# fransiskusbudi/multimodal_segmentation_project

Hardware: AMD Instinct MI355X
Metric: 3D volumes/sec (96^3, 4-class) fwd+bwd per node (higher is better)
Workload: dtype bf16; 1 GPU; UNet3D(1->4, features 16/32/64/128) 96^3 patch, per-GPU batch 2, fwd + Dice/CE loss + bwd + AdamW + metrics, dropout 0.0; global_batch=2, parallelism=dp1, hipgraph=False

## Files before the change

multimodal_segmentation_project_amd/csrc/common.h:

```cpp
#pragma once
#include <hip/hip_runtime.h>
#include <stdint.h>

typedef __bf16 bf16;
typedef __attribute__((ext_vector_type(8))) __bf16 bf16x8;
typedef __attribute__((ext_vector_type(4))) __bf16 bf16x4;
typedef __attribute__((ext_vector_type(4))) float f32x4;
typedef __attribute__((ext_vector_type(16))) float f32x16;

enum { MI3D_F32 = 0, MI3D_BF16 = 1 };

void mi3d_set_error(const char* fmt, ...);
#define MI3D_CHECK_ARG(cond, ...)                 \
    do {                                          \
        if (!(cond)) {                            \
            mi3d_set_error(__VA_ARGS__);          \
            return -1;                            \
        }                                         \
    } while (0)
#define MI3D_HIP(call)                                                                   \
    do {                                                                                 \
        hipError_t e_ = (call);                                                          \
        if (e_ != hipSuccess) {                                                          \
            mi3d_set_error("%s failed: %s (%s:%d)", #call, hipGetErrorString(e_), __FILE__, __LINE__); \
            return (int)e_;                                                              \
        }                                                                                \
    } while (0)
#define MI3D_LAUNCH_CHECK() MI3D_HIP(hipGetLastError())
#define MI3D_TRY(expr)          \
    do {                        \
        int rc_ = (expr);       \
        if (rc_ != 0) return rc_; \
    } while (0)

#define MI3D_ROUTE_LIST(X)                                                                                          \
    X(no_planar, 0)                                     \
    X(no_persist, 0)                                \
    X(no_head_loss, 0)                      \
    X(no_pool_fuse, 0)                                           \
    X(no_small_bn, 0)       \
    X(no_defer_tail, 0)                                     \
    X(no_upbwd_carry, 0)      \
    X(no_fused_bwd, 0)         \
    X(no_fused_bwd_p, 0)                                          \
    X(no_fused_bwd_big, 0)                                              \
    X(no_fused_upbwd, 0)                   \
    X(conv8, 1)                                  \
    X(no_pool_splitk, 0)     \
    X(no_pool_pair, 0)       \
    X(wide_bn, 3)            \
    X(splitk_ticket, 1)
struct Mi3dRoutes {
#define MI3D_ROUTE_FIELD(name, dflt) int name = dflt;
    MI3D_ROUTE_LIST(MI3D_ROUTE_FIELD)
#undef MI3D_ROUTE_FIELD
};
const Mi3dRoutes& mi3d_routes();

#ifdef __HIPCC__
#define MI3D_HD __host__ __device__
// ... 89 lines not shown
```

multimodal_segmentation_project_amd/csrc/conv3_mfma.hip:

```cpp
#include <stdlib.h>

#include <type_traits>

#include <hip/hip_ext.h>

#include "mfma_tile.h"
#include "ops.h"
#include "slab_sum.h"

namespace {

constexpr int BLK = 256;

MI3D_HD constexpr int ktap(int mode, int s, int h) {
    if (mode == 0) return 2 * s + h;
    if (s < 12) {
        int dz = s / 4, k = s % 4;
        return k < 3 ? dz * 9 + k * 3 + h : dz * 9 + h * 3 + 2;
    }
    if (s == 12) return h * 9 + 8;
    return h == 0 ? 26 : 27;
}

__global__ void pack_mfma_kernel(const float* __restrict__ w, int Cin, int Cout, bf16* __restrict__ wf, bf16* __restrict__ wd,
                                 int mode_f, int mode_d) {
    int64_t n = (int64_t)Cin * Cout * 28;
    for (int64_t i = (int64_t)blockIdx.x * blockDim.x + threadIdx.x; i < 2 * n; i += (int64_t)gridDim.x * blockDim.x) {
        bool dg = i >= n;
        int64_t k = dg ? i - n : i;
        int j = k & 7; int lane = (k >> 3) & 63; int64_t r = k >> 9;
        int nob = (dg ? Cin : Cout) / 16;
// ... 547 lines not shown
            }
            __syncthreads();
            bn_row_write<COB, 8, false>(red, tk_rows, bid_.x, CoutTotal, cobBase * 16);
            return;
        }
    }
    float s1[COB][4], s2[COB][4];
#pragma unroll
    for (int c = 0; c < COB; c++)
#pragma unroll
        for (int j = 0; j < 4; j++) s1[c][j] = s2[c][j] = 0.f;
#pragma unroll
    for (int r = 0; r < MBW; r++)
        conv_epilogue<T, COB, STATS, true>(acc[r], bias, y, ycs, relu, n, z0 + zs, y0, x0, hb * MBW + r, vn, g, D, H, W, cobBase, s1, s2);
    if constexpr (STATS) bn_rows_reduce<COB, 8, false>(s1, s2, red, wave, vn, g, part, bid_.x, CoutTotal, cobBase * 16);
}

template <int COB, int NCH, bool STATS, bool EXT_LDS = false>
__device__ __forceinline__ void conv3_mfma_persist_body(Bid bid_, const bf16* __restrict__ x, int xcs,
                                                        const bf16* __restrict__ wp, const float* __restrict__ bias,
                                                        bf16* __restrict__ y, int ycs, int D, int H, int W,
                                                        int tilesZ, int tilesY, int tilesX, int ntiles,
                                                        float* __restrict__ part, Halves xh, Halves yh, char* ext_lds = nullptr,
                                                        int relu = 0) {
    using T = FullTile;
    using L = LdsP<COB, NCH>;
    constexpr int TZ = T::TZ, TY = T::TY, TX = T::TX, IY = T::IY, IX = T::IX, MB = T::MB;
    static_assert(T::BX == 16 && T::IXP == IX && MB == 8, "a lane's voxel is x position vn of M-block row r; rows are not padded");
    constexpr int NVOX = T::NVOX, NIT = T::pieces(BLK);
    constexpr int CoutTotal = COB * 16;
    constexpr int NWF = NCH * 14 * COB;
    bf16* xs; bf16* wl;
    float (*red)[COB][16][2];
    if constexpr (EXT_LDS) {
        xs = reinterpret_cast<bf16*>(ext_lds + L::xs);
        wl = reinterpret_cast<bf16*>(ext_lds + L::wl);
        red = reinterpret_cast<float (*)[COB][16][2]>(ext_lds + L::red);
    } else {
        __shared__ __attribute__((aligned(16))) bf16 xs_s[(L::wl - L::xs) / 2];
        __shared__ __attribute__((aligned(16))) bf16 wl_s[(L::red - L::wl) / 2];
        __shared__ float red_s[4][COB][16][2];
        static_assert(sizeof(xs_s) + sizeof(wl_s) + sizeof(red_s) == L::bytes, "the three arrays are the layout");
        xs = xs_s; wl = wl_s; red = red_s;
    }
    int lane = threadIdx.x & 63, wave = threadIdx.x >> 6;
    int vn = lane & 15, g = lane >> 4;
    int laneOff = ((vn * 16 + (g & 1) * 8) * 2) + wave * (IY * IX * 32);
// ... 10 lines not shown
    bool lastValid = threadIdx.x + (NIT - 1) * BLK < NVOX * 2;
    unsigned pk[(NIT + 1) / 2];
#pragma unroll
    for (int i = 0; i < (NIT + 1) / 2; i++) pk[i] = 0;
#pragma unroll
    for (int it = 0; it < NIT; it++) {
        int vox = (threadIdx.x + it * BLK) >> 1;
        int ix = vox % IX, t = vox / IX, iy = t % IY, iz = t / IY;
        if (iz > 7) iz = 7;
        pk[it >> 1] |= (unsigned)(ix | (iy << 5) | (iz << 9)) << ((it & 1) * 16);
    }
    float bv[COB][4];
#pragma unroll
    for (int c = 0; c < COB; c++)
#pragma unroll
        for (int j = 0; j < 4; j++) bv[c][j] = bias ? bias[c * 16 + g * 4 + j] : 0.f;
    float s1[COB][4], s2[COB][4];
#pragma unroll
    for (int c = 0; c < COB; c++)
#pragma unroll
        for (int j = 0; j < 4; j++) s1[c][j] = s2[c][j] = 0.f;

    bf16x8 sv[NIT];
    auto tile_origin = [&](int tile, int& n, int& z0, int& y0, int& x0) {
        int tz_ = tile % tilesZ; tile /= tilesZ;
        int ty_ = tile % tilesY; tile /= tilesY;
        int tx_ = tile % tilesX; n = tile / tilesX;
        z0 = tz_ * TZ; y0 = ty_ * TY; x0 = tx_ * TX;
    };
    auto load_pieces = [&](int tile, int chunk) {
        int n, z0, y0, x0;
        tile_origin(tile, n, z0, y0, x0);
        int64_t base = ((((int64_t)n * D + (z0 - 1)) * H + (y0 - 1)) * W + (x0 - 1)) * xcs + chunk * 16 +
                       (chunk >= xh.split ? xh.delta : 0);
        const bf16* xb = x + base;
        bool interior = z0 >= 1 && z0 + TZ + 1 <= D && y0 >= 1 && y0 + TY + 1 <= H && x0 >= 1 && x0 + TX + 1 <= W;
        if (interior) {
#pragma unroll
            for (int it = 0; it < NIT; it++) {
                if (it < NIT - 1 || lastValid) sv[it] = *reinterpret_cast<const bf16x8*>(xb + rel[it]);
            }
        } else {
#pragma unroll
            for (int it = 0; it < NIT; it++) {
                unsigned c = pk[it >> 1] >> ((it & 1) * 16);
                unsigned gz = (unsigned)(z0 - 1) + ((c >> 9) & 7u), gy = (unsigned)(y0 - 1) + ((c >> 5) & 15u),
                         gx = (unsigned)(x0 - 1) + (c & 31u);
                bool inb = (it < NIT - 1 || lastValid) && gz < (unsigned)D && gy < (unsigned)H && gx < (unsigned)W;
                sv[it] = bf16x8{0, 0, 0, 0, 0, 0, 0, 0};
                if (inb) sv[it] = *reinterpret_cast<const bf16x8*>(xb + rel[it]);
            }
        }
    };

    int tile = xcd_contig(bid_.x, bid_.gx);
    if (tile < ntiles) load_pieces(tile, 0);
    for (int i = threadIdx.x; i < NWF * 64; i += BLK)
        *reinterpret_cast<bf16x8*>(wl + i * 8) = *reinterpret_cast<const bf16x8*>(wp + (int64_t)i * 8);
    for (; tile < ntiles; tile += bid_.gx) {
        f32x4 acc[MB][COB];
#pragma unroll
        for (int r = 0; r < MB; r++)
#pragma unroll
            for (int c = 0; c < COB; c++) acc[r][c] = f32x4{0.f, 0.f, 0.f, 0.f};
#pragma unroll
        for (int ch = 0; ch < NCH; ch++) {
            __syncthreads();
#pragma unroll
            for (int it = 0; it < NIT; it++) {
                int idx = threadIdx.x + it * BLK;
                if (it < NIT - 1 || idx < NVOX * 2) *reinterpret_cast<bf16x8*>(xs + idx * 8) = sv[it];
            }
            __syncthreads();
            if (ch + 1 < NCH) load_pieces(tile, ch + 1);
            else if (tile + bid_.gx < ntiles) load_pieces(tile + bid_.gx, 0);
            auto W_ = [&](int s, int c) -> bf16x8 {
                return *reinterpret_cast<const bf16x8*>(wl + ((ch * 14 + s) * COB + c) * 512 + lane * 8);
            };
            const int hx = (g >> 1) * 32;
            const int hy = (g >> 1) * (IX * 32) + 64;
            const int hz = (g >> 1) * (IY * IX * 32) + (2 * IX + 2) * 32;
            bf16x8 F[10], G[8];
#pragma unroll
            for (int row = 0; row < 10; row++) F[row] = *reinterpret_cast<const bf16x8*>(xsb + laneOff + hx + row * (IX * 32));
#pragma unroll
            for (int dz = 0; dz < 3; dz++) {
#pragma unroll
                for (int r = 0; r < 8; r++)
                    G[r] = *reinterpret_cast<const bf16x8*>(xsb + laneOff + hy + (dz * IY + r) * (IX * 32));
#pragma unroll
                for (int dy = 0; dy < 3; dy++) {
                    bf16x8 wc_[COB];
#pragma unroll
                    for (int c = 0; c < COB; c++) wc_[c] = W_(dz * 4 + dy, c);
#pragma unroll
                    for (int r = 0; r < 8; r++)
#pragma unroll
                        for (int c = 0; c < COB; c++) acc[r][c] = mfma16(wc_[c], F[r + dy], acc[r][c]);
// ... 15 lines not shown
#pragma unroll
                        for (int c = 0; c < COB; c++) acc[r][c] = mfma16(wc_[c], G[r], acc[r][c]);
                }
            }
#pragma unroll
            for (int r = 0; r < 8; r++)
                G[r] = *reinterpret_cast<const bf16x8*>(xsb + laneOff + (2 * IY * IX + 2 * IX + 2) * 32 + r * (IX * 32));
            {
                bf16x8 wc_[COB];
#pragma unroll
                for (int c = 0; c < COB; c++) wc_[c] = W_(12, c);
#pragma unroll
                for (int r = 0; r < 8; r++)
#pragma unroll
                    for (int c = 0; c < COB; c++) acc[r][c] = mfma16(wc_[c], F[r], acc[r][c]);
#pragma unroll
                for (int c = 0; c < COB; c++) wc_[c] = W_(13, c);
#pragma unroll
                for (int r = 0; r < 8; r++)
#pragma unroll
                    for (int c = 0; c < COB; c++) acc[r][c] = mfma16(wc_[c], G[r], acc[r][c]);
            }
        }
        int n, z0, y0, x0;
        tile_origin(tile, n, z0, y0, x0);
        int gz = z0 + wave, gx = x0 + vn;
        bf16* yrow = y + ((((int64_t)n * D + gz) * H + y0) * W + gx) * ycs + g * 4;
        bool okzx = gz < D && gx < W;
        if (relu & 2) {
            bf16* ywide = y + ((((int64_t)n * D + gz) * H + y0 + (g & 1)) * W + gx) * ycs + (g >> 1) * 8;
#pragma unroll
            for (int r = 0; r < MB; r += 2) {
                const bool okw = okzx && (y0 + r + (g & 1)) < H;
#pragma unroll
                for (int c = 0; c < COB; c++) {
                    bf16x4 oa, ob;
#pragma unroll
                    for (int j = 0; j < 4; j++) {
                        float va = acc[r][c][j] + bv[c][j], vb = acc[r + 1][c][j] + bv[c][j];
                        if (relu & 1) { va = fmaxf(va, 0.f); vb = fmaxf(vb, 0.f); }
                        oa[j] = (bf16)va; ob[j] = (bf16)vb;
                        if (STATS) {
                            float qa = (okzx && (y0 + r) < H) ? (float)oa[j] : 0.f, qb = (okzx && (y0 + r + 1) < H) ? (float)ob[j] : 0.f;
                            s1[c][j] += qa; s2[c][j] = fmaf(qa, qa, s2[c][j]);
                            s1[c][j] += qb; s2[c][j] = fmaf(qb, qb, s2[c][j]);
                        }
                    }
                    u32x4 w = swap_halves16(oa, ob);
                    if (okw) *reinterpret_cast<u32x4*>(ywide + (int64_t)r * W * ycs + c * 16 + (c >= yh.split ? yh.delta : 0)) = w;
                }
            }
            continue;
        }
#pragma unroll
        for (int r = 0; r < MB; r++) {
            bool ok = okzx && (y0 + r) < H;
#pragma unroll
            for (int c = 0; c < COB; c++) {
                bf16x4 o = round4_masked<STATS>(acc[r][c], bv[c], relu, ok, s1[c], s2[c]);
                if (ok) *reinterpret_cast<bf16x4*>(yrow + (int64_t)r * W * ycs + c * 16 + (c >= yh.split ? yh.delta : 0)) = o;
            }
        }
    }
    if constexpr (STATS) bn_rows_reduce<COB, 4, true>(s1, s2, red, wave, vn, g, part, bid_.x, CoutTotal, 0);
}

template <int COB, int NCH, bool STATS>
__global__ __launch_bounds__(BLK, 2) void conv3_mfma_persist_kernel(const bf16* __restrict__ x, int xcs,
                                                                    const bf16* __restrict__ wp, const float* __restrict__ bias,
                                                                    bf16* __restrict__ y, int ycs, int D, int H, int W,
                                                                    int tilesZ, int tilesY, int tilesX, int ntiles,
                                                                    float* __restrict__ part, Halves xh, Halves yh, int relu) {
    conv3_mfma_persist_body<COB, NCH, STATS>(real_bid(), x, xcs, wp, bias, y, ycs, D, H, W, tilesZ, tilesY, tilesX, ntiles, part, xh, yh,
                                             nullptr, relu);
}

inline int device_cus() {
    static const int n = [] {
        int dev = 0, v = 0;
        if (hipGetDevice(&dev) != hipSuccess || hipDeviceGetAttribute(&v, hipDeviceAttributeMultiprocessorCount, dev) != hipSuccess || v < 8)
            v = 256;
        (void)hipGetLastError();
        return v;
    }();
    return n;
}
struct TimeHook { hipEvent_t e0 = nullptr, e1 = nullptr; int kind = -1, cin = 0, cout = 0; bool armed = false, fired = false; };
static thread_local TimeHook g_hook;
inline bool time_hook_take(int kind, int cin, int cout, hipEvent_t& e0, hipEvent_t& e1) {
    if (kind < 0 || !g_hook.armed || g_hook.kind != kind || g_hook.cin != cin || g_hook.cout != cout) return false;
    e0 = g_hook.e0; e1 = g_hook.e1;
    g_hook.armed = false; g_hook.fired = true;
    return true;
}
template <auto Kernel, typename... Args>
int launch_hooked(dim3 grid, dim3 block, size_t lds, hipStream_t s, int kind, int cin, int cout, Args... args) {
    if (lds) MI3D_SET_MAX_LDS_ONCE(Kernel, lds);
    hipEvent_t e0 = nullptr, e1 = nullptr;
    if (time_hook_take(kind, cin, cout, e0, e1)) hipExtLaunchKernelGGL(Kernel, grid, block, lds, s, e0, e1, 0, args...);
    else Kernel<<<grid, block, lds, s>>>(args...);
    MI3D_LAUNCH_CHECK();
    return 0;
}

inline bool persist_ok(int Cin, int Cout, Geo g) {
    int64_t nt = (int64_t)g.N * cdiv(g.D, 4) * cdiv(g.H, 8) * cdiv(g.W, 16);
    if (Cin == 16 && Cout == 32 && nt < 1024) return false;
    return g.W >= 32 && g.H >= 16 && ((Cin == 16 && Cout == 16) || (Cin == 32 && Cout == 16) || (Cin == 16 && Cout == 32)) &&
           !mi3d_routes().no_persist;
}
inline int persist_grid(int Cin, int Cout, Geo g) {
    int64_t nt = (int64_t)g.N * cdiv(g.D, 4) * cdiv(g.H, 8) * cdiv(g.W, 16);
    int want = 2 * device_cus();
    return (int)(nt < want ? nt : want);
}

__device__ __forceinline__ void splitk_finish_body(int blk, int nblk, const float* __restrict__ part, int ksplit, int64_t M, int C,
                                                   const float* __restrict__ bias, bf16* __restrict__ y, int ycs, int relu = 0) {
    int G8 = C / 8;
    int64_t total = M * G8;
    for (int64_t idx = (int64_t)blk * BLK + threadIdx.x; idx < total; idx += (int64_t)nblk * BLK) {
        int64_t v = idx / G8;
        int c0 = (int)(idx - v * G8) * 8;
        float a[8];
#pragma unroll
        for (int j = 0; j < 8; j++) a[j] = bias ? bias[c0 + j] : 0.f;
        for (int k = 0; k < ksplit; k++) {
            const float* p = part + ((int64_t)k * M + v) * C + c0;
            f32x4 u = *reinterpret_cast<const f32x4*>(p), w = *reinterpret_cast<const f32x4*>(p + 4);
            a[0] += u[0]; a[1] += u[1]; a[2] += u[2]; a[3] += u[3]; a[4] += w[0]; a[5] += w[1]; a[6] += w[2]; a[7] += w[3];
        }
        if (relu) {
// ... 118 lines not shown
bool conv3_mfma_fuses_stats(int Cin, int Cout, Geo g) { return pick_ksplit(Cin, Cout, g) == 1; }

bool conv3_mfma_halves_ok(int Cin, int Cout, Geo g) { return persist_ok(Cin, Cout, g); }

bool conv3_mfma_ticket_ok(int Cin, int Cout, Geo g) {
    if (!mi3d_routes().splitk_ticket || mi3d_routes().conv8 == 0 || big_geo(g) || persist_ok(Cin, Cout, g)) return false;
    if (pick_ksplit(Cin, Cout, g) <= 1) return false;
    const int64_t wgs = (int64_t)g.N * cdiv(g.D, 4) * cdiv(g.H, 8) * cdiv(g.W, 8) * (Cout / (Cout % 32 == 0 ? 32 : 16));
    return wgs <= CONV3_TK_COUNTERS;
}

int conv3_mfma_fwd(const void* x, int xcs, int Cin, const void* wp, const float* bias, void* y, int ycs, int Cout, Geo g,
                   float* part, float* skws, hipStream_t s, Halves xh, Halves yh, int* ks_deferred, int relu, int split_target,
                   float* tk_rows, int* tk_count) {
    if (ks_deferred) *ks_deferred = 0;
    MI3D_CHECK_ARG(!tk_rows || (conv3_mfma_ticket_ok(Cin, Cout, g) && skws && split_target == 0), "conv3_mfma_fwd: no split-K ticket for %d->%d here", Cin, Cout);
    MI3D_CHECK_ARG((!xh.on() && !yh.on()) || persist_ok(Cin, Cout, g), "conv3_mfma_fwd: planar halves need the persistent kernel");
    MI3D_CHECK_ARG(conv3_mfma_supported(Cin, Cout, xcs, ycs), "conv3_mfma_fwd: unsupported channels %d->%d", Cin, Cout);
    MI3D_CHECK_ARG(((uintptr_t)x % 16) == 0 && ((uintptr_t)y % 8) == 0, "conv3_mfma_fwd: misaligned tensors");
    const bf16* xp = (const bf16*)x; const bf16* w = (const bf16*)wp; bf16* yp = (bf16*)y;
    bool two = Cout % 32 == 0;
    if (persist_ok(Cin, Cout, g)) {
        int tz = cdiv(g.D, 4), ty = cdiv(g.H, 8), tx = cdiv(g.W, 16), nt = g.N * tz * ty * tx, grid = persist_grid(Cin, Cout, g);
        if (ycs % 8 == 0 && ((uintptr_t)y % 16) == 0 && yh.delta % 8 == 0) relu |= 2;
        auto launch = [&](auto cob, auto nch) -> int {
            constexpr int COB = decltype(cob)::value, NCH = decltype(nch)::value;
            if (part)
                return launch_hooked<conv3_mfma_persist_kernel<COB, NCH, true>>(grid, BLK, 0, s, 2, Cin, Cout, xp, xcs, w, bias, yp, ycs, g.D, g.H, g.W,
                                                                                tz, ty, tx, nt, part, xh, yh, relu);
            return launch_hooked<conv3_mfma_persist_kernel<COB, NCH, false>>(grid, BLK, 0, s, 3, Cin, Cout, xp, xcs, w, bias, yp, ycs, g.D, g.H, g.W,
                                                                             tz, ty, tx, nt, (float*)nullptr, xh, yh, relu);
        };
        constexpr std::integral_constant<int, 1> one{};
        constexpr std::integral_constant<int, 2> two{};
        return Cin == 16 && Cout == 16 ? launch(one, one) : Cin == 32 ? launch(one, two) : launch(two, one);
    }
    int ks = skws ? pick_ksplit(Cin, Cout, g, split_target) : 1;
    if (ycs % 8 == 0 && ((uintptr_t)y % 16) == 0 && Cout % 32 == 0) relu |= 2;
    if (ks > 1) MI3D_CHECK_ARG(ycs % 8 == 0 && ((uintptr_t)y % 16) == 0, "conv3_mfma_fwd: split-K needs 16-B aligned output rows");
    if (big_geo(g)) {
        if (two) return launch_cfg<4, 8, 1, 16, 2>(xp, xcs, Cin, w, bias, yp, ycs, Cout, g, part, 1, nullptr, s, false, relu);
        return launch_cfg<4, 8, 1, 16, 1>(xp, xcs, Cin, w, bias, yp, ycs, Cout, g, part, 1, nullptr, s, false, relu);
    }
    if (tk_rows) {
        if (two) return launch_cfg<4, 2, 2, 4, 2>(xp, xcs, Cin, w, bias, yp, ycs, Cout, g, nullptr, ks, skws, s, false, 0, tk_rows, tk_count);
        return launch_cfg<4, 2, 2, 4, 1>(xp, xcs, Cin, w, bias, yp, ycs, Cout, g, nullptr, ks, skws, s, false, 0, tk_rows, tk_count);
    }
// ... 63 lines not shown
#pragma unroll
    for (int a = 0; a < CO_B; a++) dbs[a] = 0.f;
    bool do_db = (tg == 0 && bid_.z == 0);

    int ntiles = N * tilesZ * tilesY * tilesX;
    static_assert(CO_B == 1 && CI_B == 1 && BLK == 256 && WTY * WTX * 2 == BLK && WIY * WIX * 2 == 360, "staging map");
    constexpr int NA = WTZ, NXJ = 3, NXP = WIZ / 2, NB = NXP * NXJ;
    const int hv = threadIdx.x >> 1, hf = threadIdx.x & 1;
    const int a_iy = hv / WTX, a_ix = hv % WTX;
    const unsigned a_rel = (unsigned)(((a_iy * W + a_ix) * dycs + hf * 8) * 2);
    const bool b_act = threadIdx.x < 240;
    int b_iy[NXJ], b_ix[NXJ], b_iz[NXJ];
    unsigned b_rel[NXJ];
#pragma unroll
    for (int j = 0; j < NXJ; j++) {
        int v = 120 * j + (b_act ? hv : 0);
        b_iz[j] = v / (WIY * WIX);
        int r = v % (WIY * WIX);
        b_iy[j] = r / WIX;
        b_ix[j] = r % WIX;
        b_rel[j] = (unsigned)((((b_iz[j] * H + b_iy[j]) * W + b_ix[j]) * xcs + hf * 8) * 2);
    }
    bf16x8 va[NA], vb[NB];
    auto load_tile = [&](int tile) {
        int t = tile;
        int tx_ = t % tilesX; t /= tilesX;
        int ty_ = t % tilesY; t /= tilesY;
        int tz_ = t % tilesZ; int n = t / tilesZ;
        int z0 = tz_ * WTZ, y0 = ty_ * WTY, x0 = tx_ * WTX;
        const char* dyn = reinterpret_cast<const char*>(dy + ((((int64_t)n * D + z0) * H + y0) * W + x0) * dycs + co0);
        const char* xn = reinterpret_cast<const char*>(x + ci0 + ((ci0 >> 4) >= xh.split ? xh.delta : 0)) +
                         ((((int64_t)n * D + (z0 - 1)) * H + (y0 - 1)) * W + (x0 - 1)) * xcs * 2;
        const int64_t a_zs = (int64_t)H * W * dycs * 2, b_zs = (int64_t)H * W * xcs * 2;
        bool a_ok = y0 + a_iy < H && x0 + a_ix < W;
#pragma unroll
        for (int it = 0; it < NA; it++) {
            va[it] = bf16x8{0, 0, 0, 0, 0, 0, 0, 0};
            if (a_ok && z0 + it < D) va[it] = *reinterpret_cast<const bf16x8*>(dyn + it * a_zs + a_rel);
        }
        bool b_ok[NXJ];
#pragma unroll
        for (int j = 0; j < NXJ; j++)
            b_ok[j] = b_act && (unsigned)(y0 - 1 + b_iy[j]) < (unsigned)H && (unsigned)(x0 - 1 + b_ix[j]) < (unsigned)W;
#pragma unroll
        for (int pz = 0; pz < NXP; pz++)
#pragma unroll
            for (int j = 0; j < NXJ; j++) {
                vb[pz * NXJ + j] = bf16x8{0, 0, 0, 0, 0, 0, 0, 0};
                if (b_ok[j] && (unsigned)(z0 - 1 + 2 * pz + b_iz[j]) < (unsigned)D)
                    vb[pz * NXJ + j] = *reinterpret_cast<const bf16x8*>(xn + 2 * pz * b_zs + b_rel[j]);
            }
    };
    constexpr bool PF = (NT * CO_B * CI_B + NA + NB) * 4 <= 300;
    const int tile0 = xcd_tiles ? xcd_contig(sb, nsb) : sb;
    if (PF && tile0 < ntiles) load_tile(tile0);
    for (int tile = tile0; tile < ntiles; tile += nsb) {
        if (!PF) load_tile(tile);
        __syncthreads();
#pragma unroll
        for (int it = 0; it < NA; it++) *reinterpret_cast<bf16x8*>(dys + (threadIdx.x + it * BLK) * 8) = va[it];
        if (b_act) {
#pragma unroll
            for (int it = 0; it < NB; it++)
                *reinterpret_cast<bf16x8*>(xs + ((it / NXJ) * 720 + (it % NXJ) * 240 + threadIdx.x) * 8) = vb[it];
        }
        __syncthreads();
        if (PF && tile + nsb < ntiles) load_tile(tile + nsb);
        bf16x8 A[WTZ][CO_B];
#pragma unroll
        for (int z = 0; z < WTZ; z++)
#pragma unroll
            for (int a = 0; a < CO_B; a++) {
                A[z][a] = tr_frag(dysb, laneA + z * (WTY * WTX * 32) + a * (WNV * 32));
                if (do_db) {
#pragma unroll
                    for (int j = 0; j < 8; j++) dbs[a] += (float)A[z][a][j];
                }
            }
        constexpr int NBF = WIZ * NY * 3 * CI_B, PFD = 4;
        auto bfrag = [&](int t) {
            int b_ = t % CI_B, r = t / CI_B;
            int dx = r % 3; r /= 3;
            int dyi = r % NY, zz = r / NY;
            int dy = (NT == 27) ? dyi : tg;
            return tr_frag(xsb, laneB + ((zz * WIY + dy) * WIX + dx) * 32 + b_ * (WNH * 32));
        };
        bf16x8 Bq[PFD];
#pragma unroll
        for (int t = 0; t < PFD; t++) Bq[t] = bfrag(t);
#pragma unroll
// ... 67 lines not shown
};
struct FusedPArgs {
    const bf16* wx; int wxcs, wCin; const bf16* wdy; int wdycs, wCout; int tZ, tY, tX; float* slabs; int wgx, wgy, wgz; Halves wxh;
    const bf16* dxin; int dxcs_in; const bf16* dwp; bf16* dyout; int dycs_out; int ptZ, ptY, ptX, pnt, pgrid; Halves dyh;
    int N, D, H, W;
    int xcd_tiles, flags;
};
template <int COB, int NCH>
__global__ __launch_bounds__(BLK, 2) void conv3_bwd_fused_persist_kernel(FusedPArgs a) {
    extern __shared__ __attribute__((aligned(16))) char fusedp_lds[];
    int nw = a.wgx * a.wgy * a.wgz;
    int b = blockIdx.x;
    bool is_w = (b & 1) == 0;
    int idx = b >> 1;
    if (is_w) {
        if (idx >= nw) return;
        Bid v{idx % a.wgx, (idx / a.wgx) % a.wgy, idx / (a.wgx * a.wgy), a.wgx, a.wgy, a.wgz};
        conv3_wgrad_body<1, 1, 27>(v, a.wx, a.wxcs, a.wCin, a.wdy, a.wdycs, a.wCout, a.N, a.D, a.H, a.W, a.tZ, a.tY, a.tX, 1, a.slabs, a.wxh,
                                   a.xcd_tiles);
    } else {
        if (idx >= a.pgrid) return;
        Bid v{idx, 0, 0, a.pgrid, 1, 1};
        conv3_mfma_persist_body<COB, NCH, false, true>(v, a.dxin, a.dxcs_in, a.dwp, nullptr, a.dyout, a.dycs_out, a.D, a.H, a.W, a.ptZ, a.ptY,
                                                       a.ptX, a.pnt, nullptr, Halves(), a.dyh, fusedp_lds, a.flags);
    }
}

template <bool BIG, bool SPLITK>
__global__ __launch_bounds__(BLK, 2) void conv3_bwd_fused_kernel(FusedArgs a) {
    extern __shared__ __attribute__((aligned(16))) char fused_lds[];
    int nw = a.wgx * a.wgy * a.wgz, nwp = (nw + 7) & ~7;
    int nd = a.dgx * a.dgy * a.dgz;
    int b = blockIdx.x;
    bool is_w = b < nwp;
    if (!is_w) b -= nwp;
    if (is_w ? b >= nw : b >= nd) return;
    if (is_w) {
        int f = xcd_contig(b, nw), G = a.wgy * a.wgz, yz = f % G;
        Bid v{f / G, yz % a.wgy, yz / a.wgy, a.wgx, a.wgy, a.wgz};
        conv3_wgrad_body<1, 1, 27>(v, a.wx, a.wxcs, a.wCin, a.wdy, a.wdycs, a.wCout, a.N, a.D, a.H, a.W, a.tZ, a.tY, a.tX, 1, a.slabs,
                                   Halves());
    } else {
        if constexpr (BIG) {
            int f = xcd_contig(b, a.dgx * a.dgy);
            Bid v{f / a.dgy, f % a.dgy, 0, a.dgx, a.dgy, 1, true};
            conv3_mfma_body<4, 8, 1, 16, 2, false, false, true>(v, a.dxin, a.dxcs_in, a.dCin, a.dwp, nullptr, a.dyout, a.dycs_out, a.dCout,
                                                                a.D, a.H, a.W, a.dtZ, a.dtY, a.dtX, nullptr, fused_lds);
// ... 257 lines not shown
struct WgCfg { int cob, cib, nt, tg, nsb; };

inline WgCfg wgrad_cfg(int Cin, int Cout, Geo g, int target = 0) {
    WgCfg c;
    c.cob = 1;
    c.cib = 1;
    int groups = (Cout / 16) * (Cin / 16);
    int64_t ntiles = (int64_t)g.N * cdiv(g.D, WTZ) * cdiv(g.H, WTY) * cdiv(g.W, WTX);
    c.nt = 27;
    c.tg = 1;
    int64_t want = (target > 0 ? target : 2 * device_cus()) / (int64_t)groups;
    if (want < 1) want = 1;
    int64_t rounds = cdiv(ntiles, want);
    c.nsb = (int)cdiv(ntiles, rounds);
    return c;
}

template <int CO_B, int CI_B, int NT>
int launch_wgrad(const bf16* x, int xcs, int Cin, const bf16* dy, int dycs, int Cout, Geo g, float* slabs, WgCfg c,
                 hipStream_t s, Halves xh) {
    constexpr size_t lds = LdsWg<CO_B, CI_B>::bytes;
    dim3 grid((unsigned)(c.nsb * c.tg), (unsigned)(Cout / (16 * CO_B)), (unsigned)(Cin / (16 * CI_B)));
    const bool full = persist_ok(Cout, Cin, g);
    const int xcd_tiles = full ? 1 : 0;
    int pgx = 0, pgy = 0, pgz = 0;
    if (!full && c.tg == 1) {
        pgx = (int)grid.x; pgy = (int)grid.y; pgz = (int)grid.z;
        grid = dim3((unsigned)(pgx * pgy * pgz));
    }
    return launch_hooked<conv3_wgrad_mfma_kernel<CO_B, CI_B, NT>>(grid, BLK, lds, s, 1, Cin, Cout, x, xcs, Cin, dy, dycs, Cout, g.N, g.D, g.H, g.W,
                                                                  cdiv(g.D, WTZ), cdiv(g.H, WTY), cdiv(g.W, WTX), c.tg, slabs, xh, xcd_tiles,
                                                                  pgx, pgy, pgz);
}

inline int c1_nsb(Geo g) {
    int64_t ntiles = (int64_t)g.N * cdiv(g.D, WTZ) * cdiv(g.H, WTY) * cdiv(g.W, WTX);
    return (int)(ntiles < 1024 ? ntiles : 1024);
}

}

__global__ __launch_bounds__(BLK) void slab_job_kernel(SlabJob q) { slab_job_run(q, (int)blockIdx.x); }
int slab_job_launch(const SlabJob& q, hipStream_t s) {
    if (q.nblocks <= 0) return 0;
    slab_job_kernel<<<q.nblocks, BLK, 0, s>>>(q);
    MI3D_LAUNCH_CHECK();
    return 0;
// ... 3 lines not shown
                          SlabJob* pend = nullptr) {
    int64_t nW = (int64_t)Cout * Cin * 27, slab_sz = nW + Cout;
    if (pend) { *pend = slab_job_make((dW && slab_sz >= (800 << 10)) ? 2 : 1, ws, nsb, slab_sz, nW, dW, db, Cin, Cout, accumulate); return 0; }
    if (dW && slab_sz >= (800 << 10))
        slab_reduce_tile_kernel<<<(Cout / 16) * (Cin / 16) * 4, BLK, 0, s>>>(ws, nsb, slab_sz, nW, dW, db, accumulate, Cin, Cout);
    else if (slab_sz < (16 << 10))
        slab_reduce2_kernel<true, 8><<<cdiv(slab_sz, 8), BLK, 0, s>>>(ws, nsb, slab_sz, nW, dW, db, accumulate, Cin, Cout);
    else
        slab_reduce2_kernel<true, 32><<<cdiv(slab_sz, 32), BLK, 0, s>>>(ws, nsb, slab_sz, nW, dW, db, accumulate, Cin, Cout);
    MI3D_LAUNCH_CHECK();
    return 0;
}

size_t conv3_mfma_wgrad_ws_floats(int Cin, int Cout, Geo g) {
    if (Cin == 1) return (size_t)c1_nsb(g) * ((size_t)Cout * 27 + Cout);
    return (size_t)wgrad_cfg(Cin, Cout, g).nsb * ((size_t)Cout * Cin * 27 + Cout);
}

bool conv3_mfma_big_geo(Geo g) { return big_geo(g); }

int conv3_mfma_wgrad(const void* x, int xcs, int Cin, const void* dy, int dycs, int Cout, Geo g, float* dW, float* db,
                     int accumulate, float* ws, size_t ws_floats, hipStream_t s, Halves xh, SlabJob* pend, int wg_target) {
    MI3D_CHECK_ARG(conv3_mfma_supported(Cin, Cout, xcs, dycs) && dycs % 8 == 0, "conv3_mfma_wgrad: unsupported channels");
    WgCfg c = wgrad_cfg(Cin, Cout, g, wg_target);
    int64_t nW = (int64_t)Cout * Cin * 27, slab_sz = nW + Cout;
    MI3D_CHECK_ARG(ws_floats >= (size_t)c.nsb * slab_sz, "conv3_mfma_wgrad: workspace too small");
    const bf16* xp = (const bf16*)x; const bf16* dp = (const bf16*)dy;
    int rc;
    if (c.cob == 1 && c.cib == 1) rc = launch_wgrad<1, 1, 27>(xp, xcs, Cin, dp, dycs, Cout, g, ws, c, s, xh);
    else { MI3D_CHECK_ARG(false, "conv3_mfma_wgrad: no kernel for this block config"); return -1; }
    MI3D_TRY(rc);
    return wgrad_slab_sum(ws, c.nsb, Cin, Cout, dW, db, accumulate, s, pend);
}


extern "C" int mi3d_time_next_conv3_kernel(void* start_event, void* stop_event, int kind, int Cin, int Cout) {
    g_hook = TimeHook();
    if (!start_event || !stop_event) return 0;
    g_hook.e0 = (hipEvent_t)start_event; g_hook.e1 = (hipEvent_t)stop_event;
    g_hook.kind = kind; g_hook.cin = Cin; g_hook.cout = Cout; g_hook.armed = true;
    return 0;
}
extern "C" int mi3d_time_hook_fired(void) {
    const int f = g_hook.fired ? 1 : 0;
    g_hook = TimeHook();
    return f;
}

bool conv3_mfma_bwd_fused_persist_ok(int Cin, int Cout, int xcs, int dycs, Geo g) {
    return persist_ok(Cout, Cin, g) && conv3_mfma_supported(Cin, Cout, xcs, dycs) && dycs % 8 == 0 && !mi3d_routes().no_fused_bwd &&
           !mi3d_routes().no_fused_bwd_p;
}
int conv3_mfma_bwd_fused_persist(const void* x, int xcs, int Cin, const void* dy, int dycs, int Cout, const void* wp_dgrad, void* dx,
                                 int dxcs, Geo g, float* dW, float* db, int accumulate, float* wgws, size_t wgws_floats,
                                 hipStream_t s, Halves xh, Halves dxh, SlabJob* pend) {
    MI3D_CHECK_ARG(conv3_mfma_bwd_fused_persist_ok(Cin, Cout, xcs, dycs, g) && dx, "conv3_mfma_bwd_fused_persist: unsupported layer");
    int groups = (Cout / 16) * (Cin / 16);
    int64_t ntw = (int64_t)g.N * cdiv(g.D, WTZ) * cdiv(g.H, WTY) * cdiv(g.W, WTX);
    const int wcap = device_cus(), pcap = device_cus();
    int64_t want = wcap / groups; if (want < 1) want = 1;
    int64_t rounds = cdiv(ntw, want);
    int nsb = (int)cdiv(ntw, rounds);
    int64_t nW = (int64_t)Cout * Cin * 27, slab_sz = nW + Cout;
    MI3D_CHECK_ARG(wgws_floats >= (size_t)nsb * slab_sz, "conv3_mfma_bwd_fused_persist: workspace too small");
    FusedPArgs a;
    a.wx = (const bf16*)x; a.wxcs = xcs; a.wCin = Cin; a.wdy = (const bf16*)dy; a.wdycs = dycs; a.wCout = Cout;
    a.tZ = cdiv(g.D, WTZ); a.tY = cdiv(g.H, WTY); a.tX = cdiv(g.W, WTX); a.slabs = wgws;
    a.wgx = nsb; a.wgy = Cout / 16; a.wgz = Cin / 16; a.wxh = xh;
    a.dxin = (const bf16*)dy; a.dxcs_in = dycs; a.dwp = (const bf16*)wp_dgrad; a.dyout = (bf16*)dx; a.dycs_out = dxcs;
    a.ptZ = cdiv(g.D, 4); a.ptY = cdiv(g.H, 8); a.ptX = cdiv(g.W, 16); a.pnt = g.N * a.ptZ * a.ptY * a.ptX;
    a.pgrid = a.pnt < pcap ? a.pnt : pcap; a.dyh = dxh;
    a.N = g.N; a.D = g.D; a.H = g.H; a.W = g.W;
    a.xcd_tiles = 1;
    a.flags = (dxcs % 8 == 0 && ((uintptr_t)dx % 16) == 0 && dxh.delta % 8 == 0) ? 2 : 0;
    int nw = a.wgx * a.wgy * a.wgz;
    int half = nw > a.pgrid ? nw : a.pgrid;
    unsigned nblk = (unsigned)(2 * half);
    auto launch = [&](auto cob, auto nch) -> int {
        constexpr int COB = decltype(cob)::value, NCH = decltype(nch)::value;
        constexpr size_t lds = LdsP<COB, NCH>::bytes > LdsWg<1, 1>::bytes ? LdsP<COB, NCH>::bytes : LdsWg<1, 1>::bytes;
        static_assert(lds >= LdsP<COB, NCH>::bytes && lds >= LdsWg<1, 1>::bytes, "one LDS block for either body");
        return launch_hooked<conv3_bwd_fused_persist_kernel<COB, NCH>>(nblk, BLK, lds, s, 0, Cin, Cout, a);
    };
    constexpr std::integral_constant<int, 1> one{};
    constexpr std::integral_constant<int, 2> two{};
    MI3D_TRY(Cout == 16 && Cin == 16 ? launch(one, one) : Cout == 32 ? launch(one, two) : launch(two, one));
    return wgrad_slab_sum(wgws, nsb, Cin, Cout, dW, db, accumulate, s, pend);
}

bool conv3_mfma_bwd_fused_ok(int Cin, int Cout, int xcs, int dycs, int dxcs, Geo g) {
    if (big_geo(g) && (persist_ok(Cout, Cin, g) || mi3d_routes().no_fused_bwd_big)) return false;
    return Cin % 32 == 0 && conv3_mfma_supported(Cin, Cout, xcs, dycs) && dycs % 8 == 0 && dxcs % 8 == 0 &&
           !mi3d_routes().no_fused_bwd;
}

constexpr int FUSED_WGRAD_TARGET = 288;

int conv3_mfma_bwd_wg_target(int Cin, int Cout, int xcs, int dycs, int dxcs, Geo g) {
    if (conv3_mfma_bwd_fused_persist_ok(Cin, Cout, xcs, dycs, g)) return device_cus();
    if (conv3_mfma_bwd_fused_ok(Cin, Cout, xcs, dycs, dxcs, g)) return FUSED_WGRAD_TARGET;
    return 0;
}

int conv3_mfma_bwd_fused(const void* x, int xcs, int Cin, const void* dy, int dycs, int Cout, const void* wp_dgrad, void* dx,
                         int dxcs, Geo g, float* dW, float* db, int accumulate, float* wgws, size_t wgws_floats, float* skws,
                         hipStream_t s, SlabJob* pend, int* ks_deferred) {
    if (ks_deferred) *ks_deferred = 0;
    MI3D_CHECK_ARG(conv3_mfma_bwd_fused_ok(Cin, Cout, xcs, dycs, dxcs, g) && dx && ((uintptr_t)dx % 16) == 0 && skws,
                   "conv3_mfma_bwd_fused: unsupported layer %d->%d", Cin, Cout);
    WgCfg c = wgrad_cfg(Cin, Cout, g, FUSED_WGRAD_TARGET);
    int64_t nW = (int64_t)Cout * Cin * 27, slab_sz = nW + Cout;
    MI3D_CHECK_ARG(wgws_floats >= (size_t)c.nsb * slab_sz, "conv3_mfma_bwd_fused: workspace too small");
    bool big = big_geo(g);
    int ks = pick_ksplit(Cout, Cin, g, CONV3_BWD_SPLITK_TARGET);
    FusedArgs a;
    a.wx = (const bf16*)x; a.wxcs = xcs; a.wCin = Cin; a.wdy = (const bf16*)dy; a.wdycs = dycs; a.wCout = Cout;
    a.tZ = cdiv(g.D, WTZ); a.tY = cdiv(g.H, WTY); a.tX = cdiv(g.W, WTX); a.slabs = wgws;
    a.wgx = c.nsb; a.wgy = Cout / 16; a.wgz = Cin / 16;
    a.dxin = (const bf16*)dy; a.dxcs_in = dycs; a.dCin = Cout; a.dwp = (const bf16*)wp_dgrad; a.dyout = (bf16*)dx; a.dycs_out = dxcs;
    a.dCout = Cin; a.dtZ = cdiv(g.D, 4); a.dtY = cdiv(g.H, 8); a.dtX = cdiv(g.W, big ? 16 : 8); a.dpart = ks > 1 ? skws : nullptr;
    a.dgx = g.N * a.dtZ * a.dtY * a.dtX; a.dgy = Cin / 32; a.dgz = ks;
    a.N = g.N; a.D = g.D; a.H = g.H; a.W = g.W;
    constexpr size_t lds = LdsWg<1, 1>::bytes;
    static_assert(lds >= Lds4<ConvTile<4, 8, 1, 16>, 2>::bytes && lds >= Lds4<ConvTile<4, 2, 2, 4>, 2>::bytes,
                  "one LDS block for the weight-gradient body and either input-gradient body");
    unsigned nblk = (unsigned)(((a.wgx * a.wgy * a.wgz + 7) & ~7) + a.dgx * a.dgy * a.dgz);
    if (big) MI3D_TRY((launch_hooked<conv3_bwd_fused_kernel<true, false>>(nblk, BLK, lds, s, -1, 0, 0, a)));
    else if (ks > 1) MI3D_TRY((launch_hooked<conv3_bwd_fused_kernel<false, true>>(nblk, BLK, lds, s, -1, 0, 0, a)));
    else MI3D_TRY((launch_hooked<conv3_bwd_fused_kernel<false, false>>(nblk, BLK, lds, s, -1, 0, 0, a)));
    if (ks > 1 && ks_deferred) {
        *ks_deferred = ks;
        return wgrad_slab_sum(wgws, c.nsb, Cin, Cout, dW, db, accumulate, s, pend);
// ... 48 lines not shown
```

Baseline: 976.2 volumes/s.

## Walk persistent conv tiles in contiguous brick spans for cache locality

```diff
diff --git a/multimodal_segmentation_project_amd/csrc/common.h b/multimodal_segmentation_project_amd/csrc/common.h
--- a/multimodal_segmentation_project_amd/csrc/common.h
+++ b/multimodal_segmentation_project_amd/csrc/common.h
@@ -35,7 +35,7 @@
 
 #define MI3D_ROUTE_LIST(X)                                                                                          \
     X(no_planar, 0)                                     \
-    X(no_persist, 0)                                \
+    X(no_persist, 0)         \
     X(no_head_loss, 0)                      \
     X(no_pool_fuse, 0)                                           \
     X(no_small_bn, 0)       \
diff --git a/multimodal_segmentation_project_amd/csrc/conv3_mfma.hip b/multimodal_segmentation_project_amd/csrc/conv3_mfma.hip
--- a/multimodal_segmentation_project_amd/csrc/conv3_mfma.hip
+++ b/multimodal_segmentation_project_amd/csrc/conv3_mfma.hip
@@ -7,6 +7,7 @@
 #include "mfma_tile.h"
 #include "ops.h"
 #include "slab_sum.h"
+#include "tile_walk.h"
 
 namespace {
 
@@ -600,7 +601,7 @@
                                                         bf16* __restrict__ y, int ycs, int D, int H, int W,
                                                         int tilesZ, int tilesY, int tilesX, int ntiles,
                                                         float* __restrict__ part, Halves xh, Halves yh, char* ext_lds = nullptr,
-                                                        int relu = 0) {
+                                                        int relu = 0, int slots = 8) {
     using T = FullTile;
     using L = LdsP<COB, NCH>;
     constexpr int TZ = T::TZ, TY = T::TY, TX = T::TX, IY = T::IY, IX = T::IX, MB = T::MB;
@@ -657,15 +658,13 @@
         for (int j = 0; j < 4; j++) s1[c][j] = s2[c][j] = 0.f;
 
     bf16x8 sv[NIT];
+    const bool old_walk = relu & 4;
+    const WalkGeo wgeo = walk_geo(tilesZ, tilesY, tilesX);
     auto tile_origin = [&](int tile, int& n, int& z0, int& y0, int& x0) {
-        int tz_ = tile % tilesZ; tile /= tilesZ;
-        int ty_ = tile % tilesY; tile /= tilesY;
-        int tx_ = tile % tilesX; n = tile / tilesX;
-        z0 = tz_ * TZ; y0 = ty_ * TY; x0 = tx_ * TX;
+        WalkTile t = old_walk ? walk_decode_zyx(tile, wgeo) : walk_decode(tile, wgeo);
+        n = t.n; z0 = t.tz * TZ; y0 = t.ty * TY; x0 = t.tx * TX;
     };
-    auto load_pieces = [&](int tile, int chunk) {
-        int n, z0, y0, x0;
-        tile_origin(tile, n, z0, y0, x0);
+    auto load_pieces = [&](int n, int z0, int y0, int x0, int chunk) {
         int64_t base = ((((int64_t)n * D + (z0 - 1)) * H + (y0 - 1)) * W + (x0 - 1)) * xcs + chunk * 16 +
                        (chunk >= xh.split ? xh.delta : 0);
         const bf16* xb = x + base;
@@ -688,11 +687,19 @@
         }
     };
 
-    int tile = xcd_contig(bid_.x, bid_.gx);
-    if (tile < ntiles) load_pieces(tile, 0);
+    WalkSpan span = walk_span_rr(bid_.x, bid_.gx, slots, ntiles);
+    if (old_walk) span = WalkSpan{xcd_contig(bid_.x, bid_.gx), ntiles, bid_.gx};
+    int tile = span.first;
+    int n = 0, z0 = 0, y0 = 0, x0 = 0, nn = 0, nz0 = 0, ny0 = 0, nx0 = 0;
+    if (tile < span.end) {
+        tile_origin(tile, n, z0, y0, x0);
+        load_pieces(n, z0, y0, x0, 0);
+    }
     for (int i = threadIdx.x; i < NWF * 64; i += BLK)
         *reinterpret_cast<bf16x8*>(wl + i * 8) = *reinterpret_cast<const bf16x8*>(wp + (int64_t)i * 8);
-    for (; tile < ntiles; tile += bid_.gx) {
+    for (; tile < span.end; tile += span.step, n = nn, z0 = nz0, y0 = ny0, x0 = nx0) {
+        const bool has_next = tile + span.step < span.end;
+        if (has_next) tile_origin(tile + span.step, nn, nz0, ny0, nx0);
         f32x4 acc[MB][COB];
 #pragma unroll
         for (int r = 0; r < MB; r++)
@@ -707,8 +714,8 @@
                 if (it < NIT - 1 || idx < NVOX * 2) *reinterpret_cast<bf16x8*>(xs + idx * 8) = sv[it];
             }
             __syncthreads();
-            if (ch + 1 < NCH) load_pieces(tile, ch + 1);
-            else if (tile + bid_.gx < ntiles) load_pieces(tile + bid_.gx, 0);
+            if (ch + 1 < NCH) load_pieces(n, z0, y0, x0, ch + 1);
+            else if (has_next) load_pieces(nn, nz0, ny0, nx0, 0);
             auto W_ = [&](int s, int c) -> bf16x8 {
                 return *reinterpret_cast<const bf16x8*>(wl + ((ch * 14 + s) * COB + c) * 512 + lane * 8);
             };
@@ -770,8 +777,6 @@
                     for (int c = 0; c < COB; c++) acc[r][c] = mfma16(wc_[c], G[r], acc[r][c]);
             }
         }
-        int n, z0, y0, x0;
-        tile_origin(tile, n, z0, y0, x0);
         int gz = z0 + wave, gx = x0 + vn;
         bf16* yrow = y + ((((int64_t)n * D + gz) * H + y0) * W + gx) * ycs + g * 4;
         bool okzx = gz < D && gx < W;
@@ -805,7 +810,7 @@
             bool ok = okzx && (y0 + r) < H;
 #pragma unroll
             for (int c = 0; c < COB; c++) {
-                bf16x4 o = round4_masked<STATS>(acc[r][c], bv[c], relu, ok, s1[c], s2[c]);
+                bf16x4 o = round4_masked<STATS>(acc[r][c], bv[c], relu & 1, ok, s1[c], s2[c]);
                 if (ok) *reinterpret_cast<bf16x4*>(yrow + (int64_t)r * W * ycs + c * 16 + (c >= yh.split ? yh.delta : 0)) = o;
             }
         }
@@ -851,11 +856,13 @@
     return 0;
 }
 
+inline bool old_tile_walk() { return mi3d_routes().no_persist == 2; }
+inline bool tiles_ok(Geo g) { return (int64_t)g.N * cdiv(g.D, 4) * cdiv(g.H, 8) * cdiv(g.W, 16) < WALK_MAX_TILES; }
 inline bool persist_ok(int Cin, int Cout, Geo g) {
     int64_t nt = (int64_t)g.N * cdiv(g.D, 4) * cdiv(g.H, 8) * cdiv(g.W, 16);
     if (Cin == 16 && Cout == 32 && nt < 1024) return false;
     return g.W >= 32 && g.H >= 16 && ((Cin == 16 && Cout == 16) || (Cin == 32 && Cout == 16) || (Cin == 16 && Cout == 32)) &&
-           !mi3d_routes().no_persist;
+           (mi3d_routes().no_persist == 0 || mi3d_routes().no_persist == 2);
 }
 inline int persist_grid(int Cin, int Cout, Geo g) {
     int64_t nt = (int64_t)g.N * cdiv(g.D, 4) * cdiv(g.H, 8) * cdiv(g.W, 16);
@@ -1020,7 +1027,9 @@
     bool two = Cout % 32 == 0;
     if (persist_ok(Cin, Cout, g)) {
         int tz = cdiv(g.D, 4), ty = cdiv(g.H, 8), tx = cdiv(g.W, 16), nt = g.N * tz * ty * tx, grid = persist_grid(Cin, Cout, g);
+        MI3D_CHECK_ARG(tiles_ok(g), "conv3_mfma_fwd: too many tiles for the tile walk");
         if (ycs % 8 == 0 && ((uintptr_t)y % 16) == 0 && yh.delta % 8 == 0) relu |= 2;
+        if (old_tile_walk()) relu |= 4;
         auto launch = [&](auto cob, auto nch) -> int {
             constexpr int COB = decltype(cob)::value, NCH = decltype(nch)::value;
             if (part)
@@ -1130,12 +1139,10 @@
         b_rel[j] = (unsigned)((((b_iz[j] * H + b_iy[j]) * W + b_ix[j]) * xcs + hf * 8) * 2);
     }
     bf16x8 va[NA], vb[NB];
+    const WalkGeo wgeo = walk_geo(tilesZ, tilesY, tilesX);
     auto load_tile = [&](int tile) {
-        int t = tile;
-        int tx_ = t % tilesX; t /= tilesX;
-        int ty_ = t % tilesY; t /= tilesY;
-        int tz_ = t % tilesZ; int n = t / tilesZ;
-        int z0 = tz_ * WTZ, y0 = ty_ * WTY, x0 = tx_ * WTX;
+        WalkTile t = xcd_tiles == 2 ? walk_decode(tile, wgeo) : walk_decode_xyz(tile, wgeo);
+        int n = t.n, z0 = t.tz * WTZ, y0 = t.ty * WTY, x0 = t.tx * WTX;
         const char* dyn = reinterpret_cast<const char*>(dy + ((((int64_t)n * D + z0) * H + y0) * W + x0) * dycs + co0);
         const char* xn = reinterpret_cast<const char*>(x + ci0 + ((ci0 >> 4) >= xh.split ? xh.delta : 0)) +
                          ((((int64_t)n * D + (z0 - 1)) * H + (y0 - 1)) * W + (x0 - 1)) * xcs * 2;
@@ -1160,9 +1167,10 @@
             }
     };
     constexpr bool PF = (NT * CO_B * CI_B + NA + NB) * 4 <= 300;
-    const int tile0 = xcd_tiles ? xcd_contig(sb, nsb) : sb;
-    if (PF && tile0 < ntiles) load_tile(tile0);
-    for (int tile = tile0; tile < ntiles; tile += nsb) {
+    WalkSpan span{xcd_tiles ? xcd_contig(sb, nsb) : sb, ntiles, nsb};
+    if (xcd_tiles == 2) span = walk_span_slab(sb, nsb, ntiles);
+    if (PF && span.first < span.end) load_tile(span.first);
+    for (int tile = span.first; tile < span.end; tile += span.step) {
         if (!PF) load_tile(tile);
         __syncthreads();
 #pragma unroll
@@ -1173,7 +1181,7 @@
                 *reinterpret_cast<bf16x8*>(xs + ((it / NXJ) * 720 + (it % NXJ) * 240 + threadIdx.x) * 8) = vb[it];
         }
         __syncthreads();
-        if (PF && tile + nsb < ntiles) load_tile(tile + nsb);
+        if (PF && tile + span.step < span.end) load_tile(tile + span.step);
         bf16x8 A[WTZ][CO_B];
 #pragma unroll
         for (int z = 0; z < WTZ; z++)
@@ -1287,7 +1295,7 @@
         if (idx >= a.pgrid) return;
         Bid v{idx, 0, 0, a.pgrid, 1, 1};
         conv3_mfma_persist_body<COB, NCH, false, true>(v, a.dxin, a.dxcs_in, a.dwp, nullptr, a.dyout, a.dycs_out, a.D, a.H, a.W, a.ptZ, a.ptY,
-                                                       a.ptX, a.pnt, nullptr, Halves(), a.dyh, fusedp_lds, a.flags);
+                                                       a.ptX, a.pnt, nullptr, Halves(), a.dyh, fusedp_lds, a.flags, 4);
     }
 }
 
@@ -1591,7 +1599,7 @@
     constexpr size_t lds = LdsWg<CO_B, CI_B>::bytes;
     dim3 grid((unsigned)(c.nsb * c.tg), (unsigned)(Cout / (16 * CO_B)), (unsigned)(Cin / (16 * CI_B)));
     const bool full = persist_ok(Cout, Cin, g);
-    const int xcd_tiles = full ? 1 : 0;
+    const int xcd_tiles = full ? (old_tile_walk() ? 1 : 2) : 0;
     int pgx = 0, pgy = 0, pgz = 0;
     if (!full && c.tg == 1) {
         pgx = (int)grid.x; pgy = (int)grid.y; pgz = (int)grid.z;
@@ -1641,6 +1649,7 @@
 int conv3_mfma_wgrad(const void* x, int xcs, int Cin, const void* dy, int dycs, int Cout, Geo g, float* dW, float* db,
                      int accumulate, float* ws, size_t ws_floats, hipStream_t s, Halves xh, SlabJob* pend, int wg_target) {
     MI3D_CHECK_ARG(conv3_mfma_supported(Cin, Cout, xcs, dycs) && dycs % 8 == 0, "conv3_mfma_wgrad: unsupported channels");
+    MI3D_CHECK_ARG(tiles_ok(g), "conv3_mfma_wgrad: too many tiles for the tile walk");
     WgCfg c = wgrad_cfg(Cin, Cout, g, wg_target);
     int64_t nW = (int64_t)Cout * Cin * 27, slab_sz = nW + Cout;
     MI3D_CHECK_ARG(ws_floats >= (size_t)c.nsb * slab_sz, "conv3_mfma_wgrad: workspace too small");
@@ -1674,6 +1683,7 @@
                                  int dxcs, Geo g, float* dW, float* db, int accumulate, float* wgws, size_t wgws_floats,
                                  hipStream_t s, Halves xh, Halves dxh, SlabJob* pend) {
     MI3D_CHECK_ARG(conv3_mfma_bwd_fused_persist_ok(Cin, Cout, xcs, dycs, g) && dx, "conv3_mfma_bwd_fused_persist: unsupported layer");
+    MI3D_CHECK_ARG(tiles_ok(g), "conv3_mfma_bwd_fused_persist: too many tiles for the tile walk");
     int groups = (Cout / 16) * (Cin / 16);
     int64_t ntw = (int64_t)g.N * cdiv(g.D, WTZ) * cdiv(g.H, WTY) * cdiv(g.W, WTX);
     const int wcap = device_cus(), pcap = device_cus();
@@ -1690,8 +1700,9 @@
     a.ptZ = cdiv(g.D, 4); a.ptY = cdiv(g.H, 8); a.ptX = cdiv(g.W, 16); a.pnt = g.N * a.ptZ * a.ptY * a.ptX;
     a.pgrid = a.pnt < pcap ? a.pnt : pcap; a.dyh = dxh;
     a.N = g.N; a.D = g.D; a.H = g.H; a.W = g.W;
-    a.xcd_tiles = 1;
-    a.flags = (dxcs % 8 == 0 && ((uintptr_t)dx % 16) == 0 && dxh.delta % 8 == 0) ? 2 : 0;
+    const bool brick = !old_tile_walk();
+    a.xcd_tiles = brick ? 2 : 1;
+    a.flags = ((dxcs % 8 == 0 && ((uintptr_t)dx % 16) == 0 && dxh.delta % 8 == 0) ? 2 : 0) | (brick ? 0 : 4);
     int nw = a.wgx * a.wgy * a.wgz;
     int half = nw > a.pgrid ? nw : a.pgrid;
     unsigned nblk = (unsigned)(2 * half);
@@ -1727,6 +1738,7 @@
     if (ks_deferred) *ks_deferred = 0;
     MI3D_CHECK_ARG(conv3_mfma_bwd_fused_ok(Cin, Cout, xcs, dycs, dxcs, g) && dx && ((uintptr_t)dx % 16) == 0 && skws,
                    "conv3_mfma_bwd_fused: unsupported layer %d->%d", Cin, Cout);
+    MI3D_CHECK_ARG(tiles_ok(g), "conv3_mfma_bwd_fused: too many tiles for the tile walk");
     WgCfg c = wgrad_cfg(Cin, Cout, g, FUSED_WGRAD_TARGET);
     int64_t nW = (int64_t)Cout * Cin * 27, slab_sz = nW + Cout;
     MI3D_CHECK_ARG(wgws_floats >= (size_t)c.nsb * slab_sz, "conv3_mfma_bwd_fused: workspace too small");
diff --git a/multimodal_segmentation_project_amd/csrc/tile_walk.h b/multimodal_segmentation_project_amd/csrc/tile_walk.h
--- /dev/null
+++ b/multimodal_segmentation_project_amd/csrc/tile_walk.h
@@ -0,0 +1,105 @@
+#pragma once
+
+#ifdef __HIPCC__
+#define MI3D_WALK_HD __host__ __device__ __forceinline__
+#else
+#define MI3D_WALK_HD static inline
+#endif
+
+struct WalkTile { int n, tz, ty, tx; };
+
+struct WalkDiv { int d; float inv; };
+MI3D_WALK_HD WalkDiv walk_div(int d) {
+    WalkDiv w;
+    w.d = d; w.inv = 1.0f / (float)d;
+    return w;
+}
+MI3D_WALK_HD int walk_quot(int a, WalkDiv w) {
+    int q = (int)((float)a * w.inv);
+    const int r = a - q * w.d;
+    if (r < 0) q--;
+    else if (r >= w.d) q++;
+    return q;
+}
+enum { WALK_MAX_TILES = 1 << 24 };
+
+struct WalkGeo { int tZ, tY, tX; WalkDiv dZ, dY, dX, rows, pair; };
+MI3D_WALK_HD WalkGeo walk_geo(int tZ, int tY, int tX) {
+    WalkGeo g;
+    g.tZ = tZ; g.tY = tY; g.tX = tX;
+    g.dZ = walk_div(tZ); g.dY = walk_div(tY); g.dX = walk_div(tX);
+    g.rows = walk_div(tZ * tY);
+    g.pair = walk_div(2 * tZ);
+    return g;
+}
+
+MI3D_WALK_HD WalkTile walk_decode(int pos, const WalkGeo& g) {
+    WalkTile t;
+    const int row = walk_quot(pos, g.dX);
+    t.tx = pos - row * g.tX;
+    t.n = walk_quot(row, g.rows);
+    int r = row - t.n * g.rows.d;
+    const int p = walk_quot(r, g.pair);
+    r -= p * g.pair.d;
+    const bool single = 2 * p + 1 >= g.tY;
+    t.tz = single ? r : r >> 1;
+    t.ty = 2 * p + (single ? 0 : r & 1);
+    return t;
+}
+
+MI3D_WALK_HD WalkTile walk_decode_zyx(int pos, const WalkGeo& g) {
+    WalkTile t;
+    int q = walk_quot(pos, g.dZ);
+    t.tz = pos - q * g.tZ; pos = q;
+    q = walk_quot(pos, g.dY);
+    t.ty = pos - q * g.tY; pos = q;
+    t.n = walk_quot(pos, g.dX);
+    t.tx = pos - t.n * g.tX;
+    return t;
+}
+MI3D_WALK_HD WalkTile walk_decode_xyz(int pos, const WalkGeo& g) {
+    WalkTile t;
+    int q = walk_quot(pos, g.dX);
+    t.tx = pos - q * g.tX; pos = q;
+    q = walk_quot(pos, g.dY);
+    t.ty = pos - q * g.tY; pos = q;
+    t.n = walk_quot(pos, g.dZ);
+    t.tz = pos - t.n * g.tZ;
+    return t;
+}
+
+struct WalkSpan { int first, end, step; };
+
+MI3D_WALK_HD WalkSpan walk_span(int s, int S, int j, int J, int nt) {
+    const int lo = (int)((unsigned)(s * nt) / (unsigned)S), hi = (int)((unsigned)((s + 1) * nt) / (unsigned)S);
+    WalkSpan w;
+    w.first = lo + j; w.end = hi; w.step = J;
+    return w;
+}
+MI3D_WALK_HD WalkSpan walk_span_rr(int b, int n, int S, int nt) {
+    if (n < S) S = n;
+    const int s = b % S;
+    return walk_span(s, S, b / S, (n - s + S - 1) / S, nt);
+}
+
+enum { WALK_SLAB_SLOTS = 8 };
+MI3D_WALK_HD WalkSpan walk_span_slab(int sb, int nsb, int nt) { return walk_span_rr(sb, nsb, WALK_SLAB_SLOTS, nt); }
+
+#ifdef MI3D_WALK_EXPORT_C
+extern "C" {
+void mi3d_walk_decode(int order, int pos, int tZ, int tY, int tX, int* out) {
+    const WalkGeo g = walk_geo(tZ, tY, tX);
+    WalkTile t = order == 0 ? walk_decode(pos, g) : order == 1 ? walk_decode_zyx(pos, g) : walk_decode_xyz(pos, g);
+    out[0] = t.n; out[1] = t.tz; out[2] = t.ty; out[3] = t.tx;
+}
+int mi3d_walk_quot(int a, int d) { return walk_quot(a, walk_div(d)); }
+void mi3d_walk_span_rr(int b, int n, int S, int nt, int* out) {
+    WalkSpan w = walk_span_rr(b, n, S, nt);
+    out[0] = w.first; out[1] = w.end; out[2] = w.step;
+}
+void mi3d_walk_span_slab(int sb, int nsb, int nt, int* out) {
+    WalkSpan w = walk_span_slab(sb, nsb, nt);
+    out[0] = w.first; out[1] = w.end; out[2] = w.step;
+}
+}
+#endif
```

Result: no change. 982.6 volumes/s, median of 6 (+0.7%).
